# safes/RayTracing-Weekend

Hardware: AMD Instinct MI355X
Metric: Msamples/s, Cornell box 1920x1080 4096spp (higher is better)
Workload: dtype f32

## Files before the change

raytracing_weekend_amd/csrc/rtw_ahead.h:

```cpp
#pragma once
#include <stdint.h>

#include "../../include/rtw.h"

#ifndef RTW_PATH_AHEAD
#define RTW_PATH_AHEAD 2
#endif
#ifndef RTW_PATH_GATE_BOUNDS
#define RTW_PATH_GATE_BOUNDS 1
#endif
#ifndef RTW_PATH_NEE1
#define RTW_PATH_NEE1 1
#endif

namespace rtwk {

constexpr uint32_t kAheadShift = 30;
constexpr uint32_t kAheadMaxK = 3;
static_assert(RTW_PATH_AHEAD >= 0 && RTW_PATH_AHEAD <= (int)kAheadMaxK, "the count has two bits");

constexpr uint32_t ahead_blk_end(uint32_t word) { return word & ((1u << kAheadShift) - 1u); }
constexpr uint32_t ahead_count(uint32_t word) { return word >> kAheadShift; }
constexpr uint32_t ahead_pushed(uint32_t word) { return word + (1u << kAheadShift); }
constexpr uint32_t ahead_popped(uint32_t word) { return word - (1u << kAheadShift); }

constexpr uint32_t ahead_unit_end(uint32_t block0, uint32_t blk_end, uint32_t spp) {
    return (block0 + blk_end) * (uint32_t)RTW_SUM_BLOCK < spp ? (block0 + blk_end) * (uint32_t)RTW_SUM_BLOCK : spp;
// ... 10 lines not shown
```

raytracing_weekend_amd/csrc/rtw_device.h:

```cpp
#pragma once
#include <hip/hip_runtime.h>
#include <stdint.h>

#include "../../include/rtw.h"

#define RTW_DEV __device__ __forceinline__

#define RTW_MATH_FN RTW_DEV
#include "rtw_math.h"
#include "rtw_scene.h"

#ifndef RTW_SHORT_FORMS
#define RTW_SHORT_FORMS 1
#endif

namespace rtwdev {

struct v3 { float x, y, z; };

RTW_DEV v3 V(float x, float y, float z) { v3 r; r.x = x; r.y = y; r.z = z; return r; }
RTW_DEV v3 vadd(v3 a, v3 b) { return V(a.x + b.x, a.y + b.y, a.z + b.z); }
RTW_DEV v3 vsub(v3 a, v3 b) { return V(a.x - b.x, a.y - b.y, a.z - b.z); }
RTW_DEV v3 vmul(v3 a, v3 b) { return V(a.x * b.x, a.y * b.y, a.z * b.z); }
RTW_DEV v3 vscale(v3 a, float s) { return V(a.x * s, a.y * s, a.z * s); }
// ... 766 lines not shown
        v3 po, pd, mt;
        object_ray(sc, pr, o, d, ray_time, po, pd, mt);
        float t;
        if (prim_test(pr, po, pd, V(0.f, 0.f, 0.f), tmin, RTW_FLT_MAX, gather_time, g, t)) {
            if (t < best_t || (!ANY_HIT && t == best_t && best_prim >= 0 && !best_is_vol && pi < best_prim)) {
                best_t = t; best_prim = pi; best_is_vol = false;
                if (ANY_HIT) return;
            }
        }
    }
}

struct WalkRec { u32x4 q0, q1; };
RTW_DEV bool in_range(float a, uint32_t lo, uint32_t hi) { return __builtin_amdgcn_fmed3f(a, __uint_as_float(lo), __uint_as_float(hi)) == a; }

template <bool ANY_HIT>
RTW_DEV void walk_lds(const u32x4* __restrict__ w, const int n_groups, const v3 o, const v3 d, const float tmin, const float tmax, float& best_t, int& best_prim) {
    uint32_t key_hi = __float_as_uint(tmax), key_lo = 0u;
    const u32x4* xf = w + 2 * n_groups;
    const u32x4* r = w + 5 * n_groups;
    WalkRec A, B;
    A.q0 = r[0]; A.q1 = r[1];
#define RTW_RECT_TEST(R_, OK_, IK_, OA_, DA_, OB_, DB_)                                              \
    {                                                                                                \
        const float t = (__uint_as_float(R_.q1.x) - (OK_)) * (IK_);                                  \
        const float a = fma_(t, (DA_), (OA_));                                                       \
        const float b = fma_(t, (DB_), (OB_));                                                       \
        const bool hit = (t >= tmin) & in_range(a, R_.q0.x, R_.q0.y) & in_range(b, R_.q0.z, R_.q0.w); \
        if (ANY_HIT) {                                                                               \
            key_lo = (hit & (t < tmax)) ? 1u : key_lo;                                               \
        } else {                                                                                     \
            const unsigned long long key = ((unsigned long long)__float_as_uint(t) << 32) | R_.q1.y; \
            const bool take = hit & (key < (((unsigned long long)key_hi << 32) | key_lo));           \
            key_hi = take ? __float_as_uint(t) : key_hi;                                             \
            key_lo = take ? R_.q1.y : key_lo;                                                        \
        }                                                                                            \
    }
#define RTW_REC_LIST(N_, TEST_)                                                                      \
    {                                                                                                \
        int n_ = (N_);                                                                               \
        for (; n_ >= 2; n_ -= 2) {                                                                   \
            B.q0 = r[2]; B.q1 = r[3];                                                                \
            TEST_(A)                                                                                 \
            A.q0 = r[4]; A.q1 = r[5];                                                                \
            TEST_(B)                                                                                 \
            r += 4;                                                                                  \
        }                                                                                            \
        if (n_ > 0) {                                                                                \
            B.q0 = r[2]; B.q1 = r[3];                                                                \
            TEST_(A)                                                                                 \
            A = B;                                                                                   \
            r += 2;                                                                                  \
// ... 4 lines not shown
        const int g_xform = (int)__builtin_amdgcn_readfirstlane(g0.x);
        const int n_rx = (int)__builtin_amdgcn_readfirstlane(g0.z), n_ry = (int)__builtin_amdgcn_readfirstlane(g0.w);
        const int n_rz = (int)__builtin_amdgcn_readfirstlane(g1.x), n_sph = (int)__builtin_amdgcn_readfirstlane(g1.y);
        v3 oo = o, dd = d;
        if (g_xform != 0) {
            const u32x4 r0 = xf[3 * gi], r1 = xf[3 * gi + 1], r2 = xf[3 * gi + 2];
            float m[12];
            m[0] = __uint_as_float(r0.x); m[1] = __uint_as_float(r0.y); m[2] = __uint_as_float(r0.z); m[3] = __uint_as_float(r0.w);
            m[4] = __uint_as_float(r1.x); m[5] = __uint_as_float(r1.y); m[6] = __uint_as_float(r1.z); m[7] = __uint_as_float(r1.w);
            m[8] = __uint_as_float(r2.x); m[9] = __uint_as_float(r2.y); m[10] = __uint_as_float(r2.z); m[11] = __uint_as_float(r2.w);
            oo = xf_point(m, o);
            dd = xf_vector(m, d);
        }
        if (n_rx + n_ry + n_rz > 0) {
            const v3 inv = recip3(dd);
#define RTW_TEST_X(R_) RTW_RECT_TEST(R_, oo.x, inv.x, oo.y, dd.y, oo.z, dd.z)
#define RTW_TEST_Y(R_) RTW_RECT_TEST(R_, oo.y, inv.y, oo.x, dd.x, oo.z, dd.z)
#define RTW_TEST_Z(R_) RTW_RECT_TEST(R_, oo.z, inv.z, oo.x, dd.x, oo.y, dd.y)
            RTW_REC_LIST(n_rx, RTW_TEST_X)
            RTW_REC_LIST(n_ry, RTW_TEST_Y)
            RTW_REC_LIST(n_rz, RTW_TEST_Z)
#undef RTW_TEST_X
#undef RTW_TEST_Y
#undef RTW_TEST_Z
        }
#define RTW_TEST_SPH(R_)                                                                             \
        {                                                                                            \
            float t = 0.f;                                                                           \
            const bool hit = sphere_roots(oo, dd, V(__uint_as_float(R_.q0.x), __uint_as_float(R_.q0.y), __uint_as_float(R_.q0.z)), \
                                          __uint_as_float(R_.q0.w), tmin, RTW_FLT_MAX, t);           \
            if (ANY_HIT) {                                                                           \
                key_lo = (hit & (t < tmax)) ? 1u : key_lo;                                           \
            } else {                                                                                 \
                const unsigned long long key = ((unsigned long long)__float_as_uint(t) << 32) | R_.q1.y; \
                const bool take = hit & (key < (((unsigned long long)key_hi << 32) | key_lo));       \
                key_hi = take ? __float_as_uint(t) : key_hi;                                         \
                key_lo = take ? R_.q1.y : key_lo;                                                    \
            }                                                                                        \
        }
        RTW_REC_LIST(n_sph, RTW_TEST_SPH)
#undef RTW_TEST_SPH
    }
#undef RTW_REC_LIST
#undef RTW_RECT_TEST
    best_t = ANY_HIT ? tmax : __uint_as_float(key_hi);
    best_prim = (int)key_lo - 1;
}

template <class RNG, bool ANY_HIT, bool SKIP_VOLUMES>
RTW_DEV void traverse(const DScene& sc, v3 o, v3 d, float tmin, float tmax, float ray_time, float gather_time, RNG& g,
                      const TravMem& tm, float& best_t, int& best_prim) {
    if (!sc.use_bvh) {
        traverse_brute<RNG, ANY_HIT, SKIP_VOLUMES>(sc, o, d, tmin, tmax, ray_time, gather_time, g, best_t, best_prim);
        return;
    }
    best_t = tmax;
    best_prim = -1;
    bool best_is_vol = false;
    if (!SKIP_VOLUMES) {
        best_is_vol = volume_pass<RNG, ANY_HIT>(sc, o, d, tmin, ray_time, gather_time, g, best_t, best_prim);
        if (ANY_HIT && best_is_vol) return;
    }
// ... 325 lines not shown
```

raytracing_weekend_amd/csrc/rtw_hip.hip:

```cpp
#include <hip/hip_runtime.h>

#include <algorithm>
#include <cmath>
#include <cstdio>
#include <cstdlib>
#include <cstring>
#include <condition_variable>
#include <exception>
#include <mutex>
#include <new>
#include <stdexcept>
#include <string>
#include <thread>
#include <vector>

#include "../../include/rtw.h"
#include "rtw_bvh.h"
#include "rtw_scene.h"
#include "rtw_device.h"
#include "rtw_plan.h"
#include "rtw_accum_state.h"
#include "rtw_kernels.h"
#include "rtw_guides.h"
#include "rtw_cast.h"
// ... 22 lines not shown
#endif

using namespace rtwdev;
using namespace rtwk;

#ifdef RTW_SPLIT_BUILD
namespace rtwk {
#define RTW_EXT(K_) \
    extern template __global__ void K_<RTW_RNG_PHILOX, 0>(const KArgs); extern template __global__ void K_<RTW_RNG_PHILOX, 1>(const KArgs); extern template __global__ void K_<RTW_RNG_PHILOX, 2>(const KArgs); \
    extern template __global__ void K_<RTW_RNG_TEA_LCG, 0>(const KArgs); extern template __global__ void K_<RTW_RNG_TEA_LCG, 1>(const KArgs); extern template __global__ void K_<RTW_RNG_TEA_LCG, 2>(const KArgs);
RTW_EXT(k_path)
extern template __global__ void k_path<RTW_RNG_PHILOX, 1, 1>(const KArgs);
extern template __global__ void k_path<RTW_RNG_TEA_LCG, 1, 1>(const KArgs);
extern template __global__ void k_path<RTW_RNG_PHILOX, 0, 0, 0, 1>(const KArgs);
extern template __global__ void k_path<RTW_RNG_PHILOX, 0, 0, 1, 1>(const KArgs);
RTW_EXT(k_first)
RTW_EXT(k_shade)
RTW_EXT(k_bounce)
#undef RTW_EXT
extern template __global__ void k_classify<true>(const KArgs, uint32_t*, uint32_t*, uint32_t);
extern template __global__ void k_classify<false>(const KArgs, uint32_t*, uint32_t*, uint32_t);
#define RTW_EXT_LIST(R_) \
    extern template __global__ void k_path<R_, 0, 0, 1>(const KArgs); extern template __global__ void k_path<R_, 1, 0, 1>(const KArgs); \
    extern template __global__ void k_path<R_, 2, 0, 1>(const KArgs); extern template __global__ void k_path<R_, 1, 1, 1>(const KArgs); \
    extern template __global__ void k_first<R_, 0, 1>(const KArgs); extern template __global__ void k_first<R_, 1, 1>(const KArgs); \
    extern template __global__ void k_first<R_, 2, 1>(const KArgs);
RTW_EXT_LIST(RTW_RNG_PHILOX)
RTW_EXT_LIST(RTW_RNG_TEA_LCG)
#undef RTW_EXT_LIST
}
// ... 183 lines not shown

typedef void (*Kernel)(const KArgs);
int trace_bvh_mode(const DScene& sc) { return sc.stack_wide ? 0 : sc.n_lds_nodes >= sc.n_nodes ? 2 : 1; }
Kernel trace_bvh_kernel(int block, int mode) {
#define RTW_TB(B_) (mode == 0 ? k_trace_bvh<B_, 0> : mode == 1 ? k_trace_bvh<B_, 1> : k_trace_bvh<B_, 2>)
    return block == 1024 ? RTW_TB(1024) : block == 512 ? RTW_TB(512) : RTW_TB(256);
#undef RTW_TB
}

bool path_nee1(int rng_kind, const DScene& sc) {
    int gen = sc.pdf.gen;
    if (gen == RTW_PDF_MIXTURE || gen == RTW_PDF_MIXTURE_BIAS) gen = sc.pdf.p1_gen;
    return rng_kind == RTW_RNG_PHILOX && sc.has_tex == 0 && sc.estimator == RTW_EST_REFERENCE && sc.n_lights == 1 &&
           (gen == RTW_PDF_RECT_X || gen == RTW_PDF_RECT_Y || gen == RTW_PDF_RECT_Z);
}
Kernel path_kernel(int rng_kind, const DScene& sc, bool list = false) {
    const int feat = sc.has_tex, n_vol = sc.n_vol;
    if (path_nee1(rng_kind, sc)) return list ? k_path<RTW_RNG_PHILOX, 0, 0, 1, 1> : k_path<RTW_RNG_PHILOX, 0, 0, 0, 1>;
#define RTW_PK(R_, L_) (feat == 1 && n_vol > 0 ? k_path<R_, 1, 1, L_> : feat == 2 ? k_path<R_, 2, 0, L_> : feat == 1 ? k_path<R_, 1, 0, L_> : k_path<R_, 0, 0, L_>)
    if (list) return rng_kind == RTW_RNG_TEA_LCG ? RTW_PK(RTW_RNG_TEA_LCG, 1) : RTW_PK(RTW_RNG_PHILOX, 1);
    return rng_kind == RTW_RNG_TEA_LCG ? RTW_PK(RTW_RNG_TEA_LCG, 0) : RTW_PK(RTW_RNG_PHILOX, 0);
#undef RTW_PK
}
Kernel first_list_kernel(int rng_kind, int feat) {
#define RTW_FK(R_) (feat == 2 ? k_first<R_, 2, 1> : feat == 1 ? k_first<R_, 1, 1> : k_first<R_, 0, 1>)
    return rng_kind == RTW_RNG_TEA_LCG ? RTW_FK(RTW_RNG_TEA_LCG) : RTW_FK(RTW_RNG_PHILOX);
#undef RTW_FK
}

void launch(int which, int rng_kind, const KArgs& a, int grid, size_t lds, hipStream_t s, int block = kBlock, bool list = false) {
    const bool lcg = rng_kind == RTW_RNG_TEA_LCG;
    const int feat = a.sc.has_tex;
    if (list) {
        if (which == RTW_K_FIRST) hipLaunchKernelGGL(first_list_kernel(rng_kind, feat), dim3(grid), dim3(kBlock), lds, s, a);
        else hipLaunchKernelGGL(path_kernel(rng_kind, a.sc, true), dim3(grid), dim3(kBlock), lds, s, a);
        return;
    }
#define RTW_LAUNCH_SHADING_R(K_, LDS_, R_)                                                                        \
    do {                                                                                                          \
        if (feat == 2) hipLaunchKernelGGL((K_<R_, 2>), dim3(grid), dim3(kBlock), LDS_, s, a);                     \
        else if (feat == 1) hipLaunchKernelGGL((K_<R_, 1>), dim3(grid), dim3(kBlock), LDS_, s, a);                \
        else hipLaunchKernelGGL((K_<R_, 0>), dim3(grid), dim3(kBlock), LDS_, s, a);                               \
    } while (0)
#define RTW_LAUNCH_SHADING(K_, LDS_)                                                                              \
    do {                                                                                                          \
        if (lcg) RTW_LAUNCH_SHADING_R(K_, LDS_, RTW_RNG_TEA_LCG); else RTW_LAUNCH_SHADING_R(K_, LDS_, RTW_RNG_PHILOX); \
    } while (0)
    switch (which) {
    case RTW_K_FIRST: RTW_LAUNCH_SHADING(k_first, lds); break;
    case RTW_K_SHADE: RTW_LAUNCH_SHADING(k_shade, 0); break;
    case RTW_K_TRACE:
        if (a.sc.use_bvh) hipLaunchKernelGGL(trace_bvh_kernel(block, trace_bvh_mode(a.sc)), dim3(grid), dim3(block), lds, s, a);
        else if (a.sc.n_generic == 0) hipLaunchKernelGGL((k_trace<true>), dim3(grid), dim3(kBlock), lds, s, a);
        else hipLaunchKernelGGL((k_trace<false>), dim3(grid), dim3(kBlock), lds, s, a);
        break;
    case RTW_K_PATH: hipLaunchKernelGGL(path_kernel(rng_kind, a.sc), dim3(grid), dim3(kBlock), lds, s, a); break;
    default: RTW_LAUNCH_SHADING(k_bounce, lds); break;
#undef RTW_LAUNCH_SHADING
#undef RTW_LAUNCH_SHADING_R
    }
}

int fail_nothrow(rtw_ctx* c, int code, const char* msg) noexcept {
    if (c) {
        try { c->err.assign(msg); } catch (...) { c->err.clear(); }
    }
    return code;
}
void test_fault(const char* where) {
    const char* e = getenv("RTW_TEST_FAULT");
    if (!e || !*e) return;
// ... 326 lines not shown
        const PathLaunch& l = ps.part[part];
        if (l.count == 0) continue;
        KArgs a = base;
        a.stats = c->d_stats;
        a.sample0 = target.sample0;
        a.spp = target.spp_end;
        a.queue = c->d_queue + (part == 0 ? 0 : 4);
        a.order = target.order;
        a.order_counts = target.order_counts;
        a.blocksum = c->blocksum + (part == 0 ? 0 : ps.slots_coarse) * target.n_items;
        a.unit_sums = (part == 0 && unit_sums) ? 1u : 0u;
        a.n_jobs = (uint32_t)l.n_jobs; a.n_ranges = (uint32_t)l.n_ranges; a.units_per_job = (uint32_t)l.jb;
        a.block0 = target.blk0 + (uint32_t)(ps.b0 + l.first); a.n_blocks_pass = (uint32_t)l.count; a.unit_blocks = (uint32_t)l.unit_blocks;
        hipStream_t ls = part == 0 ? s : c->stream2;
        if (part == 1) HIP_TRY(c, hipStreamWaitEvent(ls, ev_a, 0));
        launch(RTW_K_PATH, target.rng_kind, a, l.grid, 0, ls, kBlock, target.list);
        log.launches++;
        if (part == 1) {
            HIP_TRY(c, hipEventRecord(ev_b, ls));
            HIP_TRY(c, hipStreamWaitEvent(s, ev_b, 0));
        }
    }
    HIP_TRY(c, log.close(tp, s));
    return RTW_OK;
}

int issue_batch(rtw_ctx* c, const WavefrontPlan& w, const Tuning& tune, KArgs a, rtw_ctx::Lane& L, size_t paths, size_t Sb, hipEvent_t ready,
                CallLog& log, bool list) {
    const size_t lds = c->info.lds_bytes;
    const uint32_t regions = w.grid_for(paths);
    HIP_TRY(c, hipStreamWaitEvent(L.st, ready, 0));
// ... 114 lines not shown
}

void apply_estimator(DScene& sc, int estimator) {
    if (estimator == RTW_EST_REFERENCE) return;
    sc.estimator = estimator; sc.has_tex = estimator == RTW_EST_MIXTURE ? 2 : 1;
    sc.ray_tmin = 1.0e-3f; sc.probe_eps = 1.0e-3f;
}

int render_path(rtw_ctx* c, const rtw_params* P, const Tuning& tune, const KArgs& base_in, float4* out, hipStream_t s, CallLog& log) {
    const size_t npix = base_in.npix;
    int rc = ensure_pool(c, 0, 0, npix, 0);
    if (rc) return rc;
    KArgs base = base_in;
    const PathCull cull = path_cull(c, P, tune, base, npix);
    log.culled_segments = (uint64_t)cull.culled_pixels * (uint64_t)P->spp;
    const int wg_per_cu = path_wg_per_cu((const void*)path_kernel(P->rng_kind, base.sc), 0, tune.path_grid_mult);
    const PathPlan plan = plan_path(tune, npix, P->spp, c->n_cu, wg_per_cu, cull.live_groups);
    if (plan.too_many_jobs) return fail(c, RTW_ERR_UNSUPPORTED, "too many k_path jobs");
    if ((rc = grow_order(c, plan.n_groups)) != RTW_OK) return rc;
    if ((rc = grow_blocksum(c, plan.need_slots * npix)) != RTW_OK) return rc;
    HIP_TRY(c, hipEventRecord(log.begin, s));
    HIP_TRY(c, hipMemsetAsync(c->accum, 0, npix * sizeof(float4), s));
    HIP_TRY(c, hipMemsetAsync(c->d_stats, 0, (kStatRows + 1) * 8 * sizeof(unsigned long long), s));
    if ((rc = classify_jobs(c, base, plan.n_groups, s)) != RTW_OK) return rc;
    const unsigned pix_grid = pixel_grid(c, npix);
    const PathTarget target{npix, c->d_order, c->d_queue + 1, false, 0u, (uint32_t)P->spp, P->rng_kind, (uint32_t)P->sample_offset};
    for (const PathPass& ps : plan.passes) {
        if (cull.live_groups == 0) break;
        if ((rc = issue_path_pass(c, log, base, ps, plan.unit_sums, target, s)) != RTW_OK) return rc;
        if (plan.unit_sums)
            hipLaunchKernelGGL(k_resolve_blocks, dim3(pix_grid), dim3(kBlock), 0, s, (const float4*)c->blocksum, c->accum, (uint32_t)npix, (uint32_t)ps.slots_coarse,
// ... 282 lines not shown
        c->adapt = nullptr; c->adapt_pix = 0;
        HIP_TRY(c, hipMalloc(&c->adapt, off[10]));
        c->adapt_pix = npix;
    }
    char* b = (char*)c->adapt;
    st.accum = (float4*)(b + off[0]); st.upart = (float4*)(b + off[1]); st.part = (float4*)(b + off[2]); st.mom = (double2*)(b + off[3]);
    st.n = (uint32_t*)(b + off[4]); st.list[0] = (uint32_t*)(b + off[5]); st.list[1] = (uint32_t*)(b + off[6]); st.err = (float*)(b + off[7]);
    st.masks = (unsigned long long*)(b + off[8]); st.offsets = (uint32_t*)(b + off[9]);
    return RTW_OK;
}

int adaptive_path_pass(rtw_ctx* c, const rtw_params* P, const Tuning& tune, const KArgs& base, const AdaptState& st, const uint32_t* list,
                       size_t n_list, int n_from, int n_to, hipStream_t s, CallLog& log) {
    Tuning t = tune;
    if (t.path_unit_blocks % (int)kSumUnitBlocks == 0) t.path_unit_blocks = 4;
    const int wg_per_cu = path_wg_per_cu((const void*)path_kernel(P->rng_kind, base.sc, true), 0, t.path_grid_mult);
    const PathPlan plan = plan_path(t, n_list, n_to - n_from, c->n_cu, wg_per_cu);
    if (plan.too_many_jobs) return fail(c, RTW_ERR_UNSUPPORTED, "too many k_path jobs");
    int rc = grow_blocksum(c, plan.need_slots * n_list);
    if (rc) return rc;
    const uint32_t blk0 = (uint32_t)n_from / kSumBlock;
    const PathTarget target{n_list, list, nullptr, true, blk0, (uint32_t)n_to, P->rng_kind, (uint32_t)P->sample_offset};
    for (const PathPass& ps : plan.passes) {
        if ((rc = issue_path_pass(c, log, base, ps, false, target, s)) != RTW_OK) return rc;
        hipLaunchKernelGGL(k_adapt_resolve_blocks, dim3(pixel_grid(c, n_list)), dim3(kBlock), 0, s, (const float4*)c->blocksum, list, (uint32_t)n_list,
                           (uint32_t)ps.nb, blk0 + (uint32_t)ps.b0, st.accum, st.upart, st.mom);
    }
    return RTW_OK;
}

int adaptive_wavefront_pass(rtw_ctx* c, const rtw_params* P, const Tuning& tune, const KArgs& base, const AdaptState& st, const uint32_t* list,
// ... 139 lines not shown
    A.flags = flags;
    const hipError_t e = hipMemsetAsync(A.slab, 0, off[5], c->stream);
    if (e != hipSuccess) { accum_free(c); return fail(c, RTW_ERR_DEVICE, std::string("rtw_accum: ") + hipGetErrorString(e)); }
    return RTW_OK;
}

int accum_add_path(rtw_ctx* c, const Tuning& tune, const KArgs& base_in, int n_from, int n_to, hipStream_t s, CallLog& log) {
    const rtw_ctx::Accum& A = c->acc;
    const rtw_params* P = &A.P;
    const size_t npix = base_in.npix;
    int rc = ensure_pool(c, 0, 0, npix, 0);
    if (rc) return rc;
    KArgs base = base_in;
    const PathCull cull = path_cull(c, P, tune, base, npix);
    log.culled_segments = (uint64_t)cull.culled_pixels * (uint64_t)(n_to - n_from);
    const int wg_per_cu = path_wg_per_cu((const void*)path_kernel(P->rng_kind, base.sc), 0, tune.path_grid_mult);
    const size_t n_groups = (npix + 63) / 64;
    if ((rc = grow_order(c, n_groups)) != RTW_OK) return rc;
    HIP_TRY(c, hipEventRecord(log.begin, s));
    HIP_TRY(c, hipMemsetAsync(c->d_stats, 0, (kStatRows + 1) * 8 * sizeof(unsigned long long), s));
    if (cull.live_groups == 0) return RTW_OK;
    if ((rc = classify_jobs(c, base, n_groups, s)) != RTW_OK) return rc;
    const unsigned pix_grid = pixel_grid(c, npix);
    const AccumRuns runs = accum_runs(accum_split(n_from, n_to, A.mom != nullptr), A.mom != nullptr);
    PathPlan plans[2];
    size_t need_slots = 0;
    for (int k = 0; k < runs.n; k++) {
        Tuning t = tune;
        if (!runs.run[k].units_ok && t.path_unit_blocks % (int)kSumUnitBlocks == 0) t.path_unit_blocks = 4;
        plans[k] = plan_path(t, npix, runs.run[k].n_to - runs.run[k].n_from, c->n_cu, wg_per_cu, cull.live_groups);
        if (plans[k].too_many_jobs) return fail(c, RTW_ERR_UNSUPPORTED, "too many k_path jobs");
// ... 1458 lines not shown
```

raytracing_weekend_amd/csrc/rtw_inst_list.hip:

```cpp
#include <hip/hip_runtime.h>

#define RTW_TEMPLATES_ONLY
#include "../../include/rtw.h"
#include "rtw_device.h"
#include "rtw_kernels.h"

namespace rtwk {
#if !defined(RTW_INST_LIST) || RTW_INST_LIST == 0
#define RTW_INST(R_) \
    template __global__ void k_path<R_, 0, 0, 1>(const KArgs); template __global__ void k_path<R_, 1, 0, 1>(const KArgs); \
    template __global__ void k_path<R_, 2, 0, 1>(const KArgs); template __global__ void k_path<R_, 1, 1, 1>(const KArgs);
#if !defined(RTW_INST_KIND) || RTW_INST_KIND == 0
RTW_INST(RTW_RNG_PHILOX)
template __global__ void k_path<RTW_RNG_PHILOX, 0, 0, 1, 1>(const KArgs);
#endif
#if !defined(RTW_INST_KIND) || RTW_INST_KIND == 1
RTW_INST(RTW_RNG_TEA_LCG)
#endif
#undef RTW_INST
#endif
#if !defined(RTW_INST_LIST) || RTW_INST_LIST == 1
#define RTW_INST(R_) \
    template __global__ void k_first<R_, 0, 1>(const KArgs); template __global__ void k_first<R_, 1, 1>(const KArgs); \
    template __global__ void k_first<R_, 2, 1>(const KArgs);
RTW_INST(RTW_RNG_PHILOX)
RTW_INST(RTW_RNG_TEA_LCG)
#undef RTW_INST
#endif
}
// ... 1 lines not shown
```

raytracing_weekend_amd/csrc/rtw_inst_path.hip:

```cpp
#include <hip/hip_runtime.h>

#define RTW_TEMPLATES_ONLY
#include "../../include/rtw.h"
#include "rtw_device.h"
#include "rtw_kernels.h"

namespace rtwk {
#define RTW_INST(K_) \
    template __global__ void K_<RTW_RNG_PHILOX, 0>(const KArgs); template __global__ void K_<RTW_RNG_PHILOX, 1>(const KArgs); template __global__ void K_<RTW_RNG_PHILOX, 2>(const KArgs); \
    template __global__ void K_<RTW_RNG_TEA_LCG, 0>(const KArgs); template __global__ void K_<RTW_RNG_TEA_LCG, 1>(const KArgs); template __global__ void K_<RTW_RNG_TEA_LCG, 2>(const KArgs);
RTW_INST(k_path)
#undef RTW_INST
template __global__ void k_path<RTW_RNG_PHILOX, 1, 1>(const KArgs);
template __global__ void k_path<RTW_RNG_TEA_LCG, 1, 1>(const KArgs);
template __global__ void k_path<RTW_RNG_PHILOX, 0, 0, 0, 1>(const KArgs);
template __global__ void k_classify<true>(const KArgs, uint32_t*, uint32_t*, uint32_t);
template __global__ void k_classify<false>(const KArgs, uint32_t*, uint32_t*, uint32_t);
}
```

raytracing_weekend_amd/csrc/rtw_kernels.h:

```cpp
#pragma once
#include "rtw_ahead.h"
#include "rtw_device.h"
#include "rtw_plan.h"

namespace rtwk {
using namespace rtwdev;

#ifndef RTW_MIN_WAVES
#define RTW_MIN_WAVES 1
#endif
#ifdef RTW_SUBPHASE_TIMERS
constexpr int kSubRows = 16, kSubWaves = 8192;
__device__ unsigned long long g_sub_cyc[kSubWaves][kSubRows];
RTW_DEV constexpr int rtw_sub_id(const char* n) {
    return n[0] != 's' || n[1] != 'a' ? 0 : n[3] == 'h' ? 1 : n[3] == 'l' && n[4] == 'a' ? 2 : n[3] == 'l' ? 3 : n[3] == 'm' ? 4 : n[3] == 'd' ? 5 : n[3] == 'i' ? 6 : n[3] == 'n' ? 7 : 0;
}
RTW_DEV void rtw_sub_stamp(int id) {
    const unsigned long long t_in = __builtin_amdgcn_s_memtime();
    if ((threadIdx.x & 63u) == 0u) {
        unsigned long long* row = g_sub_cyc[(blockIdx.x * (blockDim.x >> 6) + (threadIdx.x >> 6)) % kSubWaves];
        const unsigned long long open_id = row[14], t0 = row[15];
        if (t0 != 0ull) row[open_id] += t_in - t0;
        row[14] = (unsigned long long)id;
        __builtin_amdgcn_s_waitcnt(0);
// ... 1129 lines not shown
    }
}

#if defined(RTW_PHASE_TIMERS)
#define RTW_MARK(name) { const unsigned long long now_ = __builtin_amdgcn_s_memtime(); ph_cyc[ph_cur] += now_ - ph_t0; ph_t0 = now_; ph_cur = rtw_phase_id(name); }
RTW_DEV constexpr int rtw_phase_id(const char* n) { return n[0] == 'r' && n[2] == 'f' ? 0 : n[0] == 'r' ? 1 : n[0] == 'w' && n[5] == 'r' ? 2 : n[0] == 's' && n[6] == 'a' ? 3 : n[0] == 'w' ? 4 : 5; }
#else
#define RTW_MARK(name) asm volatile("; MARK " name)
#endif
#ifndef RTW_PATH_WAVES
#define RTW_PATH_WAVES 5
#endif
#ifndef RTW_PATH_COLD_WAVES
#define RTW_PATH_COLD_WAVES RTW_MIN_WAVES
#endif
template <int KIND, int TEX, int MEDIA5 = 0, int LIST = 0, int NEE1 = 0>
__global__ void __launch_bounds__(kBlock, TEX ? (MEDIA5 ? 5 : RTW_PATH_COLD_WAVES) : RTW_PATH_WAVES) k_path(const KArgs A) {
    RTW_NOISE_SHARED
    __shared__ u32x4 s_hitrec[kPathMaxPrims * 6];
    const uint32_t tid = threadIdx.x;
    const uint32_t* noise_lds = stage_noise<(TEX != 0)>(A.sc, s_noise);
    {
        const u32x4* src = (const u32x4*)A.sc.hitrec;
        for (uint32_t i = tid; i < (uint32_t)A.sc.n_prims * 6u; i += kBlock) s_hitrec[i] = src[i];
    }
    __shared__ float s_usum[3][kBlock];
    __shared__ PathConsts s_pc;
    if (tid == 0) {
        for (int q = 0; q < 3; q++) {
            s_pc.cam_o[q] = A.sc.cam.origin[q]; s_pc.cam_ll[q] = A.sc.cam.lower_left[q];
            s_pc.cam_h[q] = A.sc.cam.horizontal[q]; s_pc.cam_v[q] = A.sc.cam.vertical[q];
        }
// ... 126 lines not shown
        }
        RTW_MARK("walk_r");
        const float gt = TEX ? gather_time_of(A, gk) : 0.0f;
        float th = 1.e27f;
        int prim = -1;
#if RTW_PATH_GATE_BOUNDS
        bool walk_any = !bounds_test_decides(__ballot(busy && depth > 0u));
        if (!walk_any) walk_any = __ballot(busy && may_hit_scene(A.sc, o, d)) != 0ull;
        if (walk_any) {
#else
        const bool walk = busy && (depth > 0u || may_hit_scene(A.sc, o, d));
        if (__ballot(walk) != 0ull) {
#endif
            if (busy) {
                if (TEX) traverse_brute<Rng<KIND>, false, false>(A.sc, o, d, A.sc.ray_tmin, 1.e27f, ray_time, gt, g, th, prim);
                else walk_lds<false>(s_walk, A.sc.n_groups, o, d, A.sc.ray_tmin, 1.e27f, th, prim);
            }
        }
        RTW_MARK("shade_a");
#ifdef RTW_SUBPHASE_TIMERS
        rtw_sub_stamp(8);
#endif
        if (busy) {
            v3 so, sd, att, radiance;
            Nee nee;
            const int ev = shade_a<KIND, TEX, NEE1 && RTW_PATH_NEE1>(A.sc, g, o, d, gt, th, prim, so, sd, att, radiance, nee, noise_lds, nee_prev, s_hitrec, &s_pc);
            n_seg++;
#ifdef RTW_SUBPHASE_TIMERS
            rtw_sub_stamp(0);
#endif
            RTW_MARK("walk_s");
            if (nee.has) {
                float st;
                int sprim;
                if (TEX) traverse_brute<Rng<KIND>, true, false>(A.sc, so, nee.dir, nee.tmin, nee.tmax, 0.0f, gt, g, st, sprim);
                else walk_lds<true>(s_walk, A.sc.n_groups, so, nee.dir, nee.tmin, nee.tmax, st, sprim);
                n_shadow++;
                if (sprim < 0) radiance = vadd(radiance, nee.rad);
            }
            RTW_MARK("shade_b");
            alive = shade_b<KIND>(depth, A.max_depth, g, ev, so, sd, att, radiance, o, d, T, L, TEX == 2 && A.sc.estimator == RTW_EST_MIXTURE);
            depth++;
            rng_a = g.a;
            if (alive) {
                if (TEX) {
                    ray_time = (KIND == RTW_RNG_TEA_LCG || A.sc.has_motion) ? g.ray_time(depth) : 0.0f;
                    rng_b = g.b;
                }
            } else {
                usum = vadd(usum, V((L.x == L.x) ? L.x : 0.f, (L.y == L.y) ? L.y : 0.f, (L.z == L.z) ? L.z : 0.f));
                s_cur++;
                if ((s_cur % kSumBlock) == 0u || s_cur >= A.spp) {
// ... 3 lines not shown
                    const uint32_t pix = LIST ? __float_as_uint(s_usum[0][tid]) : yl_ * c_width + px;
                    const uint32_t b_done = blk;
                    blk++;
                    need = blk >= (AHEAD ? ahead_blk_end(blk_end) : blk_end) || s_cur >= A.spp;
                    float4* const bsum_base = (float4*)(((uint64_t)kc->bs_hi << 32) | kc->bs_lo);
                    const uint32_t ush = kc->unit_shift;
                    v3 prev = V(0.f, 0.f, 0.f);
                    if (ush != 0u && (b_done % kSumUnitBlocks) != 0u) prev = V(s_usum[0][tid], s_usum[1][tid], s_usum[2][tid]);
                    const v3 u = vadd(prev, usum);
                    if (ush == 0u || need || (blk % kSumUnitBlocks) == 0u) bsum_base[(size_t)(b_done >> ush) * c_npix + pix] = make_float4(u.x, u.y, u.z, 0.f);
                    else { s_usum[0][tid] = u.x; s_usum[1][tid] = u.y; s_usum[2][tid] = u.z; }
                    usum = V(0.f, 0.f, 0.f);
                }
            }
        }
    }
#ifdef RTW_PHASE_TIMERS
    RTW_MARK("refill");
    if (lane == 0) for (int q = 0; q < 6; q++) atomicAdd(&A.stats[kStatRows * 8 + q], ph_cyc[q]);
#endif
    for (int off = 32; off > 0; off >>= 1) {
        n_seg += __shfl_down(n_seg, off);
        n_shadow += __shfl_down(n_shadow, off);
    }
    if (lane == 0) {
        unsigned long long* row = stat_row(A);
        if (n_seg) { atomicAdd(&row[0], (unsigned long long)n_seg); atomicAdd(&row[2 + RTW_K_PATH], (unsigned long long)n_seg); }
        if (n_shadow) atomicAdd(&row[1], (unsigned long long)n_shadow);
    }
}

#ifndef RTW_TEMPLATES_ONLY
struct ResolveCull { int32_t x0, x1, y0, y1; uint32_t width, row0, row_stride, divw_m, divw_s1, divw_s2; };
__global__ void __launch_bounds__(kBlock) k_resolve_blocks(const float4* __restrict__ slots, float4* __restrict__ accum, uint32_t npix, uint32_t n_unit_slots,
                                                           uint32_t n_block_slots, uint32_t first_block, const ResolveCull R) {
    for (uint32_t i = blockIdx.x * blockDim.x + threadIdx.x; i < npix; i += gridDim.x * blockDim.x) {
        const uint32_t yl = fastdiv(i, R.divw_m, R.divw_s1, R.divw_s2);
        const int32_t x = (int32_t)(i - yl * R.width), y = (int32_t)(R.row0 + yl * R.row_stride);
        if (x < R.x0 || x >= R.x1 || y < R.y0 || y >= R.y1) continue;
// ... 132 lines not shown
```

raytracing_weekend_amd/csrc/rtw_scene.h:

```cpp
#pragma once
#include <stdint.h>

#include <algorithm>
#include <cmath>
#include <cstdio>
#include <cstring>
#include <string>
#include <vector>

#include "../../include/rtw.h"
#include "rtw_bvh.h"
#include "rtw_plan.h"

namespace rtwdev {

enum { HK_CONST_NORMAL = 0, HK_SPHERE = 1, HK_MOVING_SPHERE = 2, HK_SPHERE_XFORM = 3 };
struct HitRec {
    int32_t mat_type;
    int32_t bsdf_eval;
    float param;
    int32_t kind;
    float r, g, b;
    float inv_r;
    float nx, ny, nz;
// ... 5 lines not shown

struct BruteGroup {
    int32_t xform;
    int32_t first;
    int32_t n_rx, n_ry, n_rz, n_sph;
    int32_t pad0, pad1;
};
struct BruteRec {
    float a, b, c, d, e;
    int32_t prim;
    int32_t pad0, pad1;
};

constexpr int kWalkMaxWords = 400;

}

namespace rtwk {

enum SceneTable { ST_PRIMS, ST_XFORMS, ST_HITREC, ST_LIGHTS, ST_CLIGHTS, ST_NODES, ST_WNODES, ST_LEAVES, ST_ORDER, ST_GROUPS, ST_RECS, ST_TEXS, ST_TEXDATA,
                  ST_WALK, ST_COUNT };

struct SceneScalars {
    int32_t n_prims, n_tree, n_lights, sky_light, has_motion, n_groups, n_generic, n_walk_words;
    int32_t n_lds_nodes, has_tex, noise_lds_data, n_lds_leaves, cam_type;
    float bmin[3], bmax[3];
    rtw_camera cam;
    rtw_pdf pdf;
};
struct SceneInfo {
    SceneFacts facts;
    size_t lds_bytes;
    bool cull_ok;
    float cull_bmin[3], cull_bmax[3];
};
struct PreparedScene {
    std::vector<char> image;
    size_t off[ST_COUNT];
    SceneScalars sc;
    SceneInfo info;
};

namespace scene_detail {
using namespace rtwdev;

struct Tables {
    rtw_scene_header h;
    std::vector<rtw_prim> prims;
    std::vector<rtw_xform> xforms;
// ... 166 lines not shown

inline std::vector<uint32_t> walk_image(const Tables& s, const std::vector<BruteGroup>& groups, const std::vector<BruteRec>& recs) {
    static_assert(sizeof(BruteGroup) == 32 && sizeof(BruteRec) == 32, "walk image layout");
    const size_t ng = groups.size(), words = 5 * ng + 2 * recs.size() + 4;
    if (ng == 0 || words > (size_t)kWalkMaxWords) return {};
    std::vector<uint32_t> walk(words * 4, 0u);
    memcpy(walk.data(), groups.data(), ng * sizeof(BruteGroup));
    for (size_t g = 0; g < ng; g++) memcpy(&walk[(2 * ng + 3 * g) * 4], s.xforms[groups[g].xform].inv, 12 * sizeof(float));
    for (size_t i = 0; i < recs.size(); i++) {
        memcpy(&walk[(5 * ng + 2 * i) * 4], &recs[i], sizeof(BruteRec));
        walk[(5 * ng + 2 * i) * 4 + 5] = (uint32_t)recs[i].prim + 1u;
    }
    return walk;
}

inline void pad_wave_nodes(std::vector<rtwbvh::WNode>& wq4, float big) {
    const float pad = 1.0e-4f + big * (1.0f / 524288.0f);
    for (rtwbvh::WNode& w : wq4)
        for (int k = 0; k < 4; k++)
            if (w.ref[k] != rtwbvh::kQ4Empty)
                for (int a = 0; a < 3; a++) { w.box[k][a] -= pad; w.box[k][3 + a] += pad; }
}

template <class T>
void stage(PreparedScene& out, SceneTable t, const std::vector<T>& v, size_t min_elems = 0, size_t extra = 0) {
    out.off[t] = out.image.size();
    out.image.resize((out.off[t] + (std::max(v.size(), min_elems) + extra) * sizeof(T) + 255u) & ~size_t(255), 0);
    if (!v.empty()) memcpy(out.image.data() + out.off[t], v.data(), v.size() * sizeof(T));
}

// ... 57 lines not shown
    stage(out, ST_LEAVES, bvh.leaves, 1);
    stage(out, ST_ORDER, order, 1);
    stage(out, ST_GROUPS, groups, 1);
    stage(out, ST_RECS, recs, 0, 1);
    stage(out, ST_TEXS, s.texs, 1);
    stage(out, ST_TEXDATA, s.texdata, 1);
    stage(out, ST_WALK, walk, 1);

    sc.n_prims = (int)h.n_prims;
    sc.n_tree = (int)bvh.prim_order.size();
    sc.n_lights = (int)h.n_lights;
    sc.sky_light = h.sky_light;
    sc.n_groups = (int)groups.size();
    sc.n_walk_words = (int32_t)(walk.size() / 4);
    sc.has_tex = (dyn_tex || facts.n_vol > 0 || sc.n_generic > 0 || h.camera_type != RTW_CAM_PERSPECTIVE || h.camera.lens_radius != 0.0f) ? 1 : 0;
    sc.noise_lds_data = -1;
    for (uint32_t i = 0; i < h.n_prims && sc.noise_lds_data < 0; i++) {
        int ti = s.mats[s.prims[i].material].texture;
        if (ti < 0) continue;
        if (s.texs[ti].type == RTW_TEX_CHECKER) ti = s.texs[s.texs[ti].odd].type == RTW_TEX_NOISE ? s.texs[ti].odd : s.texs[ti].even;
        if (s.texs[ti].type == RTW_TEX_NOISE) sc.noise_lds_data = (int32_t)s.texs[ti].data;
    }
    {
        float diag = 0.f;
        for (int a = 0; a < 3; a++) diag += (all.mx[a] - all.mn[a]) * (all.mx[a] - all.mn[a]);
        const float pad = 0.01f * std::sqrt(diag) + 1.0f;
        for (int a = 0; a < 3; a++) { sc.bmin[a] = all.mn[a] - pad; sc.bmax[a] = all.mx[a] + pad; }
    }
    sc.cam = h.camera;
    sc.pdf = h.pdf;
// ... 7 lines not shown
```

Before: 19140.

## Compile a fully unrolled LDS primitive walk for the Cornell box list shape

Adds a compile-time scene shape: two groups with fixed counts of rects and spheres, the second transformed. The host detects when the prepared walk image matches that shape and selects a new k_path instantiation, with the existing generic walk kept as the fallback. The specialised walk unrolls every record test at compile time, removing the per-group readfirstlane, the loop control and the transform branches, and software-pipelines the LDS loads. It also replaces the per-lane segment and shadow counters and the final shuffle reduction with per-wave ballot popcounts. The cost is an extra kernel instantiation tied to one scene layout, which adds code size and may change register use.

Measured after the change: 21550, median of 6. 12.6% higher.

```diff
diff --git a/raytracing_weekend_amd/csrc/rtw_ahead.h b/raytracing_weekend_amd/csrc/rtw_ahead.h
--- a/raytracing_weekend_amd/csrc/rtw_ahead.h
+++ b/raytracing_weekend_amd/csrc/rtw_ahead.h
@@ -11,6 +11,9 @@
 #endif
 #ifndef RTW_PATH_NEE1
 #define RTW_PATH_NEE1 1
+#endif
+#ifndef RTW_PATH_SHAPE
+#define RTW_PATH_SHAPE 1
 #endif
 
 namespace rtwk {
diff --git a/raytracing_weekend_amd/csrc/rtw_device.h b/raytracing_weekend_amd/csrc/rtw_device.h
--- a/raytracing_weekend_amd/csrc/rtw_device.h
+++ b/raytracing_weekend_amd/csrc/rtw_device.h
@@ -1,6 +1,8 @@
 #pragma once
 #include <hip/hip_runtime.h>
 #include <stdint.h>
+
+#include <utility>
 
 #include "../../include/rtw.h"
 
@@ -804,13 +806,6 @@
 struct WalkRec { u32x4 q0, q1; };
 RTW_DEV bool in_range(float a, uint32_t lo, uint32_t hi) { return __builtin_amdgcn_fmed3f(a, __uint_as_float(lo), __uint_as_float(hi)) == a; }
 
-template <bool ANY_HIT>
-RTW_DEV void walk_lds(const u32x4* __restrict__ w, const int n_groups, const v3 o, const v3 d, const float tmin, const float tmax, float& best_t, int& best_prim) {
-    uint32_t key_hi = __float_as_uint(tmax), key_lo = 0u;
-    const u32x4* xf = w + 2 * n_groups;
-    const u32x4* r = w + 5 * n_groups;
-    WalkRec A, B;
-    A.q0 = r[0]; A.q1 = r[1];
 #define RTW_RECT_TEST(R_, OK_, IK_, OA_, DA_, OB_, DB_)                                              \
     {                                                                                                \
         const float t = (__uint_as_float(R_.q1.x) - (OK_)) * (IK_);                                  \
@@ -826,6 +821,87 @@
             key_lo = take ? R_.q1.y : key_lo;                                                        \
         }                                                                                            \
     }
+#define RTW_TEST_X(R_) RTW_RECT_TEST(R_, oo.x, inv.x, oo.y, dd.y, oo.z, dd.z)
+#define RTW_TEST_Y(R_) RTW_RECT_TEST(R_, oo.y, inv.y, oo.x, dd.x, oo.z, dd.z)
+#define RTW_TEST_Z(R_) RTW_RECT_TEST(R_, oo.z, inv.z, oo.x, dd.x, oo.y, dd.y)
+#define RTW_TEST_SPH(R_)                                                                             \
+    {                                                                                                \
+        float t = 0.f;                                                                               \
+        const bool hit = sphere_roots(oo, dd, V(__uint_as_float(R_.q0.x), __uint_as_float(R_.q0.y), __uint_as_float(R_.q0.z)), \
+                                      __uint_as_float(R_.q0.w), tmin, RTW_FLT_MAX, t);               \
+        if (ANY_HIT) {                                                                               \
+            key_lo = (hit & (t < tmax)) ? 1u : key_lo;                                               \
+        } else {                                                                                     \
+            const unsigned long long key = ((unsigned long long)__float_as_uint(t) << 32) | R_.q1.y; \
+            const bool take = hit & (key < (((unsigned long long)key_hi << 32) | key_lo));           \
+            key_hi = take ? __float_as_uint(t) : key_hi;                                             \
+            key_lo = take ? R_.q1.y : key_lo;                                                        \
+        }                                                                                            \
+    }
+RTW_DEV void walk_xform(const u32x4* __restrict__ xg, const v3 o, const v3 d, v3& oo, v3& dd) {
+    const u32x4 r0 = xg[0], r1 = xg[1], r2 = xg[2];
+    float m[12];
+    m[0] = __uint_as_float(r0.x); m[1] = __uint_as_float(r0.y); m[2] = __uint_as_float(r0.z); m[3] = __uint_as_float(r0.w);
+    m[4] = __uint_as_float(r1.x); m[5] = __uint_as_float(r1.y); m[6] = __uint_as_float(r1.z); m[7] = __uint_as_float(r1.w);
+    m[8] = __uint_as_float(r2.x); m[9] = __uint_as_float(r2.y); m[10] = __uint_as_float(r2.z); m[11] = __uint_as_float(r2.w);
+    oo = xf_point(m, o);
+    dd = xf_vector(m, d);
+}
+
+template <int... I, class F>
+RTW_DEV void walk_each(std::integer_sequence<int, I...>, F&& f) { (f(std::integral_constant<int, I>{}), ...); }
+template <bool ANY_HIT, int SHAPE>
+RTW_DEV void walk_lds_shape(const u32x4* __restrict__ w, const v3 o, const v3 d, const float tmin, const float tmax, float& best_t, int& best_prim) {
+    static_assert(SHAPE == WALK_SHAPE_CORNELL, "a compiled list shape");
+    constexpr WalkShape S = kShapeCornell;
+    constexpr int NG = S.n_groups, NR = walk_shape_recs(S, NG);
+    typedef uint32_t u32x2 __attribute__((ext_vector_type(2)));
+    uint32_t key_hi = __float_as_uint(tmax), key_lo = 0u;
+    uint32_t base = 0u;
+    asm volatile("" : "+v"(base));
+    const u32x4* r = (const u32x4*)((const char*)(w + 5 * NG) + base);
+    const u32x4* xf = r - 3 * NG;
+    WalkRec R[2];
+#define RTW_WALK_LOAD(I_)                                                                            \
+    {                                                                                                \
+        const u32x2 h_ = *(const u32x2*)(r + 2 * (I_) + 1);                                          \
+        R[(I_) & 1].q0 = r[2 * (I_)];                                                                \
+        R[(I_) & 1].q1 = u32x4{h_.x, h_.y, 0u, 0u};                                                  \
+    }
+    RTW_WALK_LOAD(0)
+    v3 oo = o, dd = d, inv = o;
+    walk_each(std::make_integer_sequence<int, NR>{}, [&](auto ri_) {
+        constexpr int ri = decltype(ri_)::value;
+        constexpr int gi = walk_shape_group(S, ri), kind = walk_shape_kind(S, ri);
+        if constexpr (ri == walk_shape_recs(S, gi)) {
+            if constexpr (S.g[gi].xform) walk_xform(xf + 3 * gi, o, d, oo, dd);
+            else { oo = o; dd = d; }
+            if constexpr (S.g[gi].n[0] + S.g[gi].n[1] + S.g[gi].n[2] > 0) inv = recip3(dd);
+        }
+        if constexpr (ri + 1 < NR) RTW_WALK_LOAD(ri + 1)
+        const WalkRec C = R[ri & 1];
+        if constexpr (kind == 0) RTW_TEST_X(C)
+        else if constexpr (kind == 1) RTW_TEST_Y(C)
+        else if constexpr (kind == 2) RTW_TEST_Z(C)
+        else RTW_TEST_SPH(C)
+        if constexpr (kind == 3 || ri + 1 == NR || walk_shape_kind(S, ri + 1) == 3 || walk_shape_group(S, ri + 1) != gi) {
+            if (ANY_HIT) asm volatile("" : "+v"(key_lo));
+            else asm volatile("" : "+v"(key_hi), "+v"(key_lo));
+        }
+    });
+#undef RTW_WALK_LOAD
+    best_t = ANY_HIT ? tmax : __uint_as_float(key_hi);
+    best_prim = (int)key_lo - 1;
+}
+
+template <bool ANY_HIT, int SHAPE = 0>
+RTW_DEV void walk_lds(const u32x4* __restrict__ w, const int n_groups, const v3 o, const v3 d, const float tmin, const float tmax, float& best_t, int& best_prim) {
+    if constexpr (SHAPE != 0) { walk_lds_shape<ANY_HIT, SHAPE>(w, o, d, tmin, tmax, best_t, best_prim); return; }
+    uint32_t key_hi = __float_as_uint(tmax), key_lo = 0u;
+    const u32x4* xf = w + 2 * n_groups;
+    const u32x4* r = w + 5 * n_groups;
+    WalkRec A, B;
+    A.q0 = r[0]; A.q1 = r[1];
 #define RTW_REC_LIST(N_, TEST_)                                                                      \
     {                                                                                                \
         int n_ = (N_);                                                                               \
@@ -860,38 +936,21 @@
         }
         if (n_rx + n_ry + n_rz > 0) {
             const v3 inv = recip3(dd);
-#define RTW_TEST_X(R_) RTW_RECT_TEST(R_, oo.x, inv.x, oo.y, dd.y, oo.z, dd.z)
-#define RTW_TEST_Y(R_) RTW_RECT_TEST(R_, oo.y, inv.y, oo.x, dd.x, oo.z, dd.z)
-#define RTW_TEST_Z(R_) RTW_RECT_TEST(R_, oo.z, inv.z, oo.x, dd.x, oo.y, dd.y)
             RTW_REC_LIST(n_rx, RTW_TEST_X)
             RTW_REC_LIST(n_ry, RTW_TEST_Y)
             RTW_REC_LIST(n_rz, RTW_TEST_Z)
+        }
+        RTW_REC_LIST(n_sph, RTW_TEST_SPH)
+    }
+#undef RTW_REC_LIST
+    best_t = ANY_HIT ? tmax : __uint_as_float(key_hi);
+    best_prim = (int)key_lo - 1;
+}
+#undef RTW_TEST_SPH
 #undef RTW_TEST_X
 #undef RTW_TEST_Y
 #undef RTW_TEST_Z
-        }
-#define RTW_TEST_SPH(R_)                                                                             \
-        {                                                                                            \
-            float t = 0.f;                                                                           \
-            const bool hit = sphere_roots(oo, dd, V(__uint_as_float(R_.q0.x), __uint_as_float(R_.q0.y), __uint_as_float(R_.q0.z)), \
-                                          __uint_as_float(R_.q0.w), tmin, RTW_FLT_MAX, t);           \
-            if (ANY_HIT) {                                                                           \
-                key_lo = (hit & (t < tmax)) ? 1u : key_lo;                                           \
-            } else {                                                                                 \
-                const unsigned long long key = ((unsigned long long)__float_as_uint(t) << 32) | R_.q1.y; \
-                const bool take = hit & (key < (((unsigned long long)key_hi << 32) | key_lo));       \
-                key_hi = take ? __float_as_uint(t) : key_hi;                                         \
-                key_lo = take ? R_.q1.y : key_lo;                                                    \
-            }                                                                                        \
-        }
-        RTW_REC_LIST(n_sph, RTW_TEST_SPH)
-#undef RTW_TEST_SPH
-    }
-#undef RTW_REC_LIST
 #undef RTW_RECT_TEST
-    best_t = ANY_HIT ? tmax : __uint_as_float(key_hi);
-    best_prim = (int)key_lo - 1;
-}
 
 template <class RNG, bool ANY_HIT, bool SKIP_VOLUMES>
 RTW_DEV void traverse(const DScene& sc, v3 o, v3 d, float tmin, float tmax, float ray_time, float gather_time, RNG& g,
diff --git a/raytracing_weekend_amd/csrc/rtw_hip.hip b/raytracing_weekend_amd/csrc/rtw_hip.hip
--- a/raytracing_weekend_amd/csrc/rtw_hip.hip
+++ b/raytracing_weekend_amd/csrc/rtw_hip.hip
@@ -60,6 +60,8 @@
 extern template __global__ void k_path<RTW_RNG_TEA_LCG, 1, 1>(const KArgs);
 extern template __global__ void k_path<RTW_RNG_PHILOX, 0, 0, 0, 1>(const KArgs);
 extern template __global__ void k_path<RTW_RNG_PHILOX, 0, 0, 1, 1>(const KArgs);
+extern template __global__ void k_path<RTW_RNG_PHILOX, 0, 0, 0, 1, WALK_SHAPE_CORNELL>(const KArgs);
+extern template __global__ void k_path<RTW_RNG_PHILOX, 0, 0, 1, 1, WALK_SHAPE_CORNELL>(const KArgs);
 RTW_EXT(k_first)
 RTW_EXT(k_shade)
 RTW_EXT(k_bounce)
@@ -273,9 +275,12 @@
     return rng_kind == RTW_RNG_PHILOX && sc.has_tex == 0 && sc.estimator == RTW_EST_REFERENCE && sc.n_lights == 1 &&
            (gen == RTW_PDF_RECT_X || gen == RTW_PDF_RECT_Y || gen == RTW_PDF_RECT_Z);
 }
-Kernel path_kernel(int rng_kind, const DScene& sc, bool list = false) {
+Kernel path_kernel(int rng_kind, const DScene& sc, int walk_shape, bool list = false) {
     const int feat = sc.has_tex, n_vol = sc.n_vol;
-    if (path_nee1(rng_kind, sc)) return list ? k_path<RTW_RNG_PHILOX, 0, 0, 1, 1> : k_path<RTW_RNG_PHILOX, 0, 0, 0, 1>;
+    if (path_nee1(rng_kind, sc)) {
+        if (walk_shape == WALK_SHAPE_CORNELL) return list ? k_path<RTW_RNG_PHILOX, 0, 0, 1, 1, WALK_SHAPE_CORNELL> : k_path<RTW_RNG_PHILOX, 0, 0, 0, 1, WALK_SHAPE_CORNELL>;
+        return list ? k_path<RTW_RNG_PHILOX, 0, 0, 1, 1> : k_path<RTW_RNG_PHILOX, 0, 0, 0, 1>;
+    }
 #define RTW_PK(R_, L_) (feat == 1 && n_vol > 0 ? k_path<R_, 1, 1, L_> : feat == 2 ? k_path<R_, 2, 0, L_> : feat == 1 ? k_path<R_, 1, 0, L_> : k_path<R_, 0, 0, L_>)
     if (list) return rng_kind == RTW_RNG_TEA_LCG ? RTW_PK(RTW_RNG_TEA_LCG, 1) : RTW_PK(RTW_RNG_PHILOX, 1);
     return rng_kind == RTW_RNG_TEA_LCG ? RTW_PK(RTW_RNG_TEA_LCG, 0) : RTW_PK(RTW_RNG_PHILOX, 0);
@@ -287,12 +292,12 @@
 #undef RTW_FK
 }
 
-void launch(int which, int rng_kind, const KArgs& a, int grid, size_t lds, hipStream_t s, int block = kBlock, bool list = false) {
+void launch(int which, int rng_kind, const KArgs& a, int grid, size_t lds, hipStream_t s, int block = kBlock, bool list = false, int walk_shape = 0) {
     const bool lcg = rng_kind == RTW_RNG_TEA_LCG;
     const int feat = a.sc.has_tex;
     if (list) {
         if (which == RTW_K_FIRST) hipLaunchKernelGGL(first_list_kernel(rng_kind, feat), dim3(grid), dim3(kBlock), lds, s, a);
-        else hipLaunchKernelGGL(path_kernel(rng_kind, a.sc, true), dim3(grid), dim3(kBlock), lds, s, a);
+        else hipLaunchKernelGGL(path_kernel(rng_kind, a.sc, walk_shape, true), dim3(grid), dim3(kBlock), lds, s, a);
         return;
     }
 #define RTW_LAUNCH_SHADING_R(K_, LDS_, R_)                                                                        \
@@ -313,7 +318,7 @@
         else if (a.sc.n_generic == 0) hipLaunchKernelGGL((k_trace<true>), dim3(grid), dim3(kBlock), lds, s, a);
         else hipLaunchKernelGGL((k_trace<false>), dim3(grid), dim3(kBlock), lds, s, a);
         break;
-    case RTW_K_PATH: hipLaunchKernelGGL(path_kernel(rng_kind, a.sc), dim3(grid), dim3(kBlock), lds, s, a); break;
+    case RTW_K_PATH: hipLaunchKernelGGL(path_kernel(rng_kind, a.sc, walk_shape), dim3(grid), dim3(kBlock), lds, s, a); break;
     default: RTW_LAUNCH_SHADING(k_bounce, lds); break;
 #undef RTW_LAUNCH_SHADING
 #undef RTW_LAUNCH_SHADING_R
@@ -670,7 +675,7 @@
         a.block0 = target.blk0 + (uint32_t)(ps.b0 + l.first); a.n_blocks_pass = (uint32_t)l.count; a.unit_blocks = (uint32_t)l.unit_blocks;
         hipStream_t ls = part == 0 ? s : c->stream2;
         if (part == 1) HIP_TRY(c, hipStreamWaitEvent(ls, ev_a, 0));
-        launch(RTW_K_PATH, target.rng_kind, a, l.grid, 0, ls, kBlock, target.list);
+        launch(RTW_K_PATH, target.rng_kind, a, l.grid, 0, ls, kBlock, target.list, c->info.walk_shape);
         log.launches++;
         if (part == 1) {
             HIP_TRY(c, hipEventRecord(ev_b, ls));
@@ -815,7 +820,7 @@
     KArgs base = base_in;
     const PathCull cull = path_cull(c, P, tune, base, npix);
     log.culled_segments = (uint64_t)cull.culled_pixels * (uint64_t)P->spp;
-    const int wg_per_cu = path_wg_per_cu((const void*)path_kernel(P->rng_kind, base.sc), 0, tune.path_grid_mult);
+    const int wg_per_cu = path_wg_per_cu((const void*)path_kernel(P->rng_kind, base.sc, c->info.walk_shape), 0, tune.path_grid_mult);
     const PathPlan plan = plan_path(tune, npix, P->spp, c->n_cu, wg_per_cu, cull.live_groups);
     if (plan.too_many_jobs) return fail(c, RTW_ERR_UNSUPPORTED, "too many k_path jobs");
     if ((rc = grow_order(c, plan.n_groups)) != RTW_OK) return rc;
@@ -1128,7 +1133,7 @@
                        size_t n_list, int n_from, int n_to, hipStream_t s, CallLog& log) {
     Tuning t = tune;
     if (t.path_unit_blocks % (int)kSumUnitBlocks == 0) t.path_unit_blocks = 4;
-    const int wg_per_cu = path_wg_per_cu((const void*)path_kernel(P->rng_kind, base.sc, true), 0, t.path_grid_mult);
+    const int wg_per_cu = path_wg_per_cu((const void*)path_kernel(P->rng_kind, base.sc, c->info.walk_shape, true), 0, t.path_grid_mult);
     const PathPlan plan = plan_path(t, n_list, n_to - n_from, c->n_cu, wg_per_cu);
     if (plan.too_many_jobs) return fail(c, RTW_ERR_UNSUPPORTED, "too many k_path jobs");
     int rc = grow_blocksum(c, plan.need_slots * n_list);
@@ -1298,7 +1303,7 @@
     KArgs base = base_in;
     const PathCull cull = path_cull(c, P, tune, base, npix);
     log.culled_segments = (uint64_t)cull.culled_pixels * (uint64_t)(n_to - n_from);
-    const int wg_per_cu = path_wg_per_cu((const void*)path_kernel(P->rng_kind, base.sc), 0, tune.path_grid_mult);
+    const int wg_per_cu = path_wg_per_cu((const void*)path_kernel(P->rng_kind, base.sc, c->info.walk_shape), 0, tune.path_grid_mult);
     const size_t n_groups = (npix + 63) / 64;
     if ((rc = grow_order(c, n_groups)) != RTW_OK) return rc;
     HIP_TRY(c, hipEventRecord(log.begin, s));
diff --git a/raytracing_weekend_amd/csrc/rtw_inst_list.hip b/raytracing_weekend_amd/csrc/rtw_inst_list.hip
--- a/raytracing_weekend_amd/csrc/rtw_inst_list.hip
+++ b/raytracing_weekend_amd/csrc/rtw_inst_list.hip
@@ -13,6 +13,7 @@
 #if !defined(RTW_INST_KIND) || RTW_INST_KIND == 0
 RTW_INST(RTW_RNG_PHILOX)
 template __global__ void k_path<RTW_RNG_PHILOX, 0, 0, 1, 1>(const KArgs);
+template __global__ void k_path<RTW_RNG_PHILOX, 0, 0, 1, 1, WALK_SHAPE_CORNELL>(const KArgs);
 #endif
 #if !defined(RTW_INST_KIND) || RTW_INST_KIND == 1
 RTW_INST(RTW_RNG_TEA_LCG)
diff --git a/raytracing_weekend_amd/csrc/rtw_inst_path.hip b/raytracing_weekend_amd/csrc/rtw_inst_path.hip
--- a/raytracing_weekend_amd/csrc/rtw_inst_path.hip
+++ b/raytracing_weekend_amd/csrc/rtw_inst_path.hip
@@ -14,6 +14,7 @@
 template __global__ void k_path<RTW_RNG_PHILOX, 1, 1>(const KArgs);
 template __global__ void k_path<RTW_RNG_TEA_LCG, 1, 1>(const KArgs);
 template __global__ void k_path<RTW_RNG_PHILOX, 0, 0, 0, 1>(const KArgs);
+template __global__ void k_path<RTW_RNG_PHILOX, 0, 0, 0, 1, WALK_SHAPE_CORNELL>(const KArgs);
 template __global__ void k_classify<true>(const KArgs, uint32_t*, uint32_t*, uint32_t);
 template __global__ void k_classify<false>(const KArgs, uint32_t*, uint32_t*, uint32_t);
 }
diff --git a/raytracing_weekend_amd/csrc/rtw_kernels.h b/raytracing_weekend_amd/csrc/rtw_kernels.h
--- a/raytracing_weekend_amd/csrc/rtw_kernels.h
+++ b/raytracing_weekend_amd/csrc/rtw_kernels.h
@@ -1167,8 +1167,10 @@
 #ifndef RTW_PATH_COLD_WAVES
 #define RTW_PATH_COLD_WAVES RTW_MIN_WAVES
 #endif
-template <int KIND, int TEX, int MEDIA5 = 0, int LIST = 0, int NEE1 = 0>
+template <int KIND, int TEX, int MEDIA5 = 0, int LIST = 0, int NEE1 = 0, int SHAPE = 0>
 __global__ void __launch_bounds__(kBlock, TEX ? (MEDIA5 ? 5 : RTW_PATH_COLD_WAVES) : RTW_PATH_WAVES) k_path(const KArgs A) {
+    static_assert(SHAPE == 0 || (NEE1 && !TEX), "the fixed-shape walks belong to the one-light instantiation");
+    constexpr int WSHAPE = RTW_PATH_SHAPE ? SHAPE : 0;
     RTW_NOISE_SHARED
     __shared__ u32x4 s_hitrec[kPathMaxPrims * 6];
     const uint32_t tid = threadIdx.x;
@@ -1325,18 +1327,20 @@
 #endif
             if (busy) {
                 if (TEX) traverse_brute<Rng<KIND>, false, false>(A.sc, o, d, A.sc.ray_tmin, 1.e27f, ray_time, gt, g, th, prim);
-                else walk_lds<false>(s_walk, A.sc.n_groups, o, d, A.sc.ray_tmin, 1.e27f, th, prim);
+                else walk_lds<false, WSHAPE>(s_walk, A.sc.n_groups, o, d, A.sc.ray_tmin, 1.e27f, th, prim);
             }
         }
         RTW_MARK("shade_a");
 #ifdef RTW_SUBPHASE_TIMERS
         rtw_sub_stamp(8);
 #endif
+        bool probed = false;
+        if constexpr (WSHAPE != 0) n_seg += (uint32_t)__popcll(__ballot(busy));
         if (busy) {
             v3 so, sd, att, radiance;
             Nee nee;
             const int ev = shade_a<KIND, TEX, NEE1 && RTW_PATH_NEE1>(A.sc, g, o, d, gt, th, prim, so, sd, att, radiance, nee, noise_lds, nee_prev, s_hitrec, &s_pc);
-            n_seg++;
+            if constexpr (WSHAPE == 0) n_seg++;
 #ifdef RTW_SUBPHASE_TIMERS
             rtw_sub_stamp(0);
 #endif
@@ -1345,8 +1349,9 @@
                 float st;
                 int sprim;
                 if (TEX) traverse_brute<Rng<KIND>, true, false>(A.sc, so, nee.dir, nee.tmin, nee.tmax, 0.0f, gt, g, st, sprim);
-                else walk_lds<true>(s_walk, A.sc.n_groups, so, nee.dir, nee.tmin, nee.tmax, st, sprim);
-                n_shadow++;
+                else walk_lds<true, WSHAPE>(s_walk, A.sc.n_groups, so, nee.dir, nee.tmin, nee.tmax, st, sprim);
+                if constexpr (WSHAPE == 0) n_shadow++;
+                else probed = true;
                 if (sprim < 0) radiance = vadd(radiance, nee.rad);
             }
             RTW_MARK("shade_b");
@@ -1380,15 +1385,17 @@
                 }
             }
         }
+        if constexpr (WSHAPE != 0) n_shadow += (uint32_t)__popcll(__ballot(probed));
     }
 #ifdef RTW_PHASE_TIMERS
     RTW_MARK("refill");
     if (lane == 0) for (int q = 0; q < 6; q++) atomicAdd(&A.stats[kStatRows * 8 + q], ph_cyc[q]);
 #endif
-    for (int off = 32; off > 0; off >>= 1) {
-        n_seg += __shfl_down(n_seg, off);
-        n_shadow += __shfl_down(n_shadow, off);
-    }
+    if constexpr (WSHAPE == 0)
+        for (int off = 32; off > 0; off >>= 1) {
+            n_seg += __shfl_down(n_seg, off);
+            n_shadow += __shfl_down(n_shadow, off);
+        }
     if (lane == 0) {
         unsigned long long* row = stat_row(A);
         if (n_seg) { atomicAdd(&row[0], (unsigned long long)n_seg); atomicAdd(&row[2 + RTW_K_PATH], (unsigned long long)n_seg); }
diff --git a/raytracing_weekend_amd/csrc/rtw_scene.h b/raytracing_weekend_amd/csrc/rtw_scene.h
--- a/raytracing_weekend_amd/csrc/rtw_scene.h
+++ b/raytracing_weekend_amd/csrc/rtw_scene.h
@@ -43,6 +43,35 @@
 
 constexpr int kWalkMaxWords = 400;
 
+struct WalkShapeGroup { bool xform; int n[4]; };
+struct WalkShape { int n_groups; WalkShapeGroup g[2]; };
+enum { WALK_SHAPE_NONE = 0, WALK_SHAPE_CORNELL = 1 };
+constexpr WalkShape kShapeCornell = {2, {{false, {2, 3, 1, 1}}, {true, {2, 2, 2, 0}}}};
+constexpr int walk_shape_recs(const WalkShape& s, int n_groups) {
+    int n = 0;
+    for (int g = 0; g < n_groups; g++) for (int k = 0; k < 4; k++) n += s.g[g].n[k];
+    return n;
+}
+constexpr int walk_shape_group(const WalkShape& s, int ri) {
+    int g = 0;
+    while (g + 1 < s.n_groups && ri >= walk_shape_recs(s, g + 1)) g++;
+    return g;
+}
+constexpr int walk_shape_kind(const WalkShape& s, int ri) {
+    const int g = walk_shape_group(s, ri);
+    int k = 0, first = walk_shape_recs(s, g);
+    while (k < 3 && ri >= first + s.g[g].n[k]) first += s.g[g].n[k++];
+    return k;
+}
+static_assert(5 * kShapeCornell.n_groups + 2 * walk_shape_recs(kShapeCornell, kShapeCornell.n_groups) + 4 <= kWalkMaxWords, "a compiled shape has a walk image");
+constexpr bool walk_shape_is(const WalkShape& s, const BruteGroup* groups, size_t n_groups) {
+    if (n_groups != (size_t)s.n_groups) return false;
+    for (int g = 0; g < s.n_groups; g++) {
+        const BruteGroup& G = groups[g];
+        if ((G.xform != 0) != s.g[g].xform || G.n_rx != s.g[g].n[0] || G.n_ry != s.g[g].n[1] || G.n_rz != s.g[g].n[2] || G.n_sph != s.g[g].n[3]) return false;
+    }
+    return true;
+}
 }
 
 namespace rtwk {
@@ -62,6 +91,7 @@
     size_t lds_bytes;
     bool cull_ok;
     float cull_bmin[3], cull_bmax[3];
+    int walk_shape;
 };
 struct PreparedScene {
     std::vector<char> image;
@@ -258,6 +288,10 @@
     return walk;
 }
 
+inline int walk_shape(const std::vector<BruteGroup>& groups) {
+    return walk_shape_is(kShapeCornell, groups.data(), groups.size()) ? WALK_SHAPE_CORNELL : WALK_SHAPE_NONE;
+}
+
 inline void pad_wave_nodes(std::vector<rtwbvh::WNode>& wq4, float big) {
     const float pad = 1.0e-4f + big * (1.0f / 524288.0f);
     for (rtwbvh::WNode& w : wq4)
@@ -345,6 +379,7 @@
     sc.n_groups = (int)groups.size();
     sc.n_walk_words = (int32_t)(walk.size() / 4);
     sc.has_tex = (dyn_tex || facts.n_vol > 0 || sc.n_generic > 0 || h.camera_type != RTW_CAM_PERSPECTIVE || h.camera.lens_radius != 0.0f) ? 1 : 0;
+    out.info.walk_shape = (walk.empty() || sc.has_tex != 0) ? WALK_SHAPE_NONE : walk_shape(groups);
     sc.noise_lds_data = -1;
     for (uint32_t i = 0; i < h.n_prims && sc.noise_lds_data < 0; i++) {
         int ti = s.mats[s.prims[i].material].texture;
```
